# frobelbest/BANet

Measured on AMD Instinct MI355X. Metric: LM iterations/sec (2-frame 640x480 5-level dense BA, 128-coeff depth basis, batch 32), higher is better.
Workload: dtype f32 (SYRK: fp32 operands as bf16x3 / scaled fp16x2 pieces, fp32 accumulate, <= 2e-7 per entry; roofline.syrk_form)

## Files before the change

banet_amd/csrc/gather128s.hip:

```cpp
#include <cstdlib>

#include "quad_common.hpp"
#include "strip_plan.hpp"
static_assert(banet::kStripSegW == banet::kStripW && banet::kStripSegH == banet::kStripH && banet::kStripMinW == banet::kWinTex, "plan.hpp sizes the strip launch by these");

#ifndef BANET_STRIP_OPT_DEFAULT
#define BANET_STRIP_OPT_DEFAULT 0
#endif

namespace banet {

constexpr int kC128s = 128;
constexpr int kSBlock = 128;
constexpr int kSWaves = kSBlock / kWave;
constexpr int kWinFloats = kWinRows * kWinTex * 32;
constexpr int kWinPitchF = kWinTex * 32;

__device__ __forceinline__ int write_lane(int v, int l, int old) { return lane_id() == l ? v : old; }

struct StripLaneEnv {
  int modev, ytv, ybv;
  int ctlv, yfv;
  int ringv;
  __device__ __forceinline__ int mode(int r) const { return __builtin_amdgcn_readlane(modev, r); }
  __device__ __forceinline__ int yt(int r) const { return __builtin_amdgcn_readlane(ytv, r); }
  __device__ __forceinline__ int yb(int r) const { return __builtin_amdgcn_readlane(ybv, r); }
  __device__ __forceinline__ void set_step(int r, int ctl, int yfirst) {
    ctlv = write_lane(ctl, r, ctlv);
    yfv = write_lane(yfirst, r, yfv);
  }
  __device__ __forceinline__ int ring_get(int i) const { return __builtin_amdgcn_readlane(ringv, i); }
  __device__ __forceinline__ void ring_set(int i, int v) { ringv = write_lane(v, i, ringv); }
};

#ifndef BANET_STRIP_NT
#define BANET_STRIP_NT 0
#endif
#if BANET_STRIP_NT >= 2
#define BANET_WIN_NT_ " nt"
#else
#define BANET_WIN_NT_ ""
#endif
__device__ __forceinline__ void glds16(const float* gbase, unsigned voff_bytes, unsigned lds_dst) {
  unsigned keep;
  asm volatile("s_mov_b32 %0, m0\n\ts_mov_b32 m0, %3\n\ts_nop 0\n\tglobal_load_lds_dwordx4 %1, %2" BANET_WIN_NT_ "\n\ts_mov_b32 m0, %0"
               : "=&s"(keep)
               : "v"(voff_bytes), "s"(gbase), "s"(lds_dst)
               : "memory");
}
__device__ __forceinline__ void glds_row(const float* gbase, unsigned v0, unsigned v1, unsigned v2, unsigned lds_dst,
                                         unsigned long long mask3) {
  unsigned keep;
  unsigned long long keepx;
  asm volatile(
      "s_mov_b32 %0, m0\n\ts_mov_b32 m0, %6\n\ts_nop 0\n\t"
      "global_load_lds_dwordx4 %2, %5" BANET_WIN_NT_ "\n\t"
      "global_load_lds_dwordx4 %3, %5 offset:1024" BANET_WIN_NT_ "\n\t"
      "s_mov_b64 %1, exec\n\ts_mov_b64 exec, %7\n\t"
      "global_load_lds_dwordx4 %4, %5 offset:2048" BANET_WIN_NT_ "\n\t"
      "s_mov_b64 exec, %1\n\ts_mov_b32 m0, %0"
      : "=&s"(keep), "=&s"(keepx)
      : "v"(v0), "v"(v1), "v"(v2), "s"(gbase), "s"(lds_dst), "s"(mask3)
      : "memory");
}
template <int N>
__device__ __forceinline__ void wait_vm() {
  asm volatile("s_waitcnt vmcnt(%0)" ::"n"(N) : "memory");
}
__device__ __forceinline__ void wait_vmcnt(int n) {
  if (n >= 8) {
    if (n >= 12) {
      if (n >= 14) wait_vm<14>();
      else wait_vm<12>();
    } else {
      if (n >= 10) wait_vm<10>();
      else wait_vm<8>();
    }
  } else {
    if (n >= 4) {
      if (n >= 6) wait_vm<6>();
      else wait_vm<4>();
    } else {
      if (n >= 2) wait_vm<2>();
      else wait_vm<0>();
    }
  }
}
static_assert(kMaxWait == 15, "wait_vmcnt implements counts up to 15");

constexpr int kStripVgprs = 224;
#if BANET_STRIP_NT >= 1
#define BANET_SRC_NT_ " nt"
#else
#define BANET_SRC_NT_ ""
#endif
#define BANET_SRC_ISSUE_(A0, A1, A2, A3, voff, rs, soff)                                                            \
  asm volatile("buffer_load_dwordx4 v[" #A0 ":" #A3 "], %0, %1, %2 offen" BANET_SRC_NT_ ::"v"(voff), "s"(rs), "s"(soff) \
               : "memory", "v" #A0, "v" #A1, "v" #A2, "v" #A3)
#define BANET_SRC_READ_(A0, A1, A2, A3, d)                                                                          \
  asm volatile("v_mov_b32 %0, v" #A0 "\n\tv_mov_b32 %1, v" #A1 "\n\tv_mov_b32 %2, v" #A2 "\n\tv_mov_b32 %3, v" #A3 \
               : "=v"(d.x), "=v"(d.y), "=v"(d.z), "=v"(d.w))
template <int SLOT, int T>
__device__ __forceinline__ void src_issue(unsigned voff, __amdgpu_buffer_rsrc_t rs, unsigned soff) {
  if constexpr (SLOT == 0 && T == 0) BANET_SRC_ISSUE_(224, 225, 226, 227, voff, rs, soff);
  if constexpr (SLOT == 0 && T == 1) BANET_SRC_ISSUE_(228, 229, 230, 231, voff, rs, soff);
  if constexpr (SLOT == 1 && T == 0) BANET_SRC_ISSUE_(232, 233, 234, 235, voff, rs, soff);
  if constexpr (SLOT == 1 && T == 1) BANET_SRC_ISSUE_(236, 237, 238, 239, voff, rs, soff);
  if constexpr (SLOT == 2 && T == 0) BANET_SRC_ISSUE_(240, 241, 242, 243, voff, rs, soff);
  if constexpr (SLOT == 2 && T == 1) BANET_SRC_ISSUE_(244, 245, 246, 247, voff, rs, soff);
  if constexpr (SLOT == 3 && T == 0) BANET_SRC_ISSUE_(248, 249, 250, 251, voff, rs, soff);
  if constexpr (SLOT == 3 && T == 1) BANET_SRC_ISSUE_(252, 253, 254, 255, voff, rs, soff);
}
template <int SLOT, int T>
__device__ __forceinline__ float4 src_read() {
  float4 d;
  if constexpr (SLOT == 0 && T == 0) BANET_SRC_READ_(224, 225, 226, 227, d);
  if constexpr (SLOT == 0 && T == 1) BANET_SRC_READ_(228, 229, 230, 231, d);
  if constexpr (SLOT == 1 && T == 0) BANET_SRC_READ_(232, 233, 234, 235, d);
  if constexpr (SLOT == 1 && T == 1) BANET_SRC_READ_(236, 237, 238, 239, d);
  if constexpr (SLOT == 2 && T == 0) BANET_SRC_READ_(240, 241, 242, 243, d);
  if constexpr (SLOT == 2 && T == 1) BANET_SRC_READ_(244, 245, 246, 247, d);
  if constexpr (SLOT == 3 && T == 0) BANET_SRC_READ_(248, 249, 250, 251, d);
  if constexpr (SLOT == 3 && T == 1) BANET_SRC_READ_(252, 253, 254, 255, d);
  return d;
}
template <int V>
struct IC {
  static constexpr int value = V;
};

extern __shared__ __attribute__((aligned(16))) float sDynS[];
constexpr int kSWaveLdsFloats = kWinFloats + kC128s;
inline size_t strip_fp_lds_bytes(int pairs, int nch) { return ((size_t)pairs * kSWaveLdsFloats + (size_t)nch * 64 + 4) * sizeof(float); }

template <int KV4, int NCH, bool FP, int OPT = 0>
__global__ __launch_bounds__(FP ? 512 : kSBlock, 2) __attribute__((amdgpu_num_vgpr(kStripVgprs / 2))) void ba_gather128s_kernel(const GatherArgs a) {
  constexpr bool kPipe = (OPT & 1) != 0, kM0Row = (OPT & 2) != 0;
  constexpr int SEGH = 4 * NCH;
  constexpr int NH = (NCH + 3) / 4;
  constexpr int CPG = NCH < 4 ? NCH : 4;
  __shared__ __attribute__((aligned(16))) float sWinS[FP ? 1 : kSWaves][FP ? 4 : kWinFloats];
  __shared__ __attribute__((aligned(16))) float sScrS[FP ? 1 : kSWaves][FP ? 4 : kC128s];
  const banet_level_t& lv = a.lv;
  const int b = blockIdx.y;
  if (a.active != nullptr && a.active[(size_t)b * a.active_stride] == 0) return;
  const int lane = threadIdx.x & 63;
  const int w = wave_id();
  [[maybe_unused]] const int nw = FP ? a.pairs : kSWaves;
  float* const sWinW = FP ? sDynS + (size_t)w * kSWaveLdsFloats : &sWinS[FP ? 0 : w][0];
  float* const sScrW = FP ? sWinW + kWinFloats : &sScrS[FP ? 0 : w][0];
  [[maybe_unused]] float* const sDep = sDynS + (size_t)nw * kSWaveLdsFloats;
  [[maybe_unused]] int* const sItem = reinterpret_cast<int*>(sDep + NCH * 64);
  const int N = lv.N, K = lv.K, H = lv.H, W = lv.W;
  constexpr int C = kC128s;
  const float* __restrict__ src_b = lv.src + (size_t)b * N * C;
  const float* __restrict__ dep_b = lv.depth + (size_t)b * N;
  const float* __restrict__ bas_b = KV4 ? lv.basis + (size_t)b * N * K : nullptr;
  const int nitems = a.tiles, segs_y = a.tiles_y;
  const int pc = lane >> 2, oc = lane & 3, hA = (lane >> 3) & 1;
  const int jA = 4 * hA + oc, jB = 4 * (1 - hA) + oc;
  const int half = lane >> 5, li = lane & 31;
  const unsigned win_base = (unsigned)(uintptr_t)(__attribute__((address_space(3))) float*)sWinW;
  const unsigned dma_off = (unsigned)((lane >> 3) * 512 + (lane & 7) * 16);
  const unsigned srcA_off = (unsigned)(pc * 512 + jA * 16), srcB_off = (unsigned)(pc * 512 + jB * 16);
  StripRowStat* sStat = reinterpret_cast<StripRowStat*>(sScrW);

  float wreg[KV4 ? KV4 : 1][4];
  if constexpr (KV4 > 0) {
#pragma unroll
    for (int kc = 0; kc < KV4; ++kc)
#pragma unroll
      for (int e = 0; e < 4; ++e) {
        const int k = kc * 128 + li * 4 + e;
        wreg[kc][e] = (k < K) ? a.Wc[(size_t)b * K + k] : 0.f;
      }
  }
  [[maybe_unused]] const auto rs_src = __builtin_amdgcn_make_buffer_rsrc(const_cast<float*>(src_b), 0, N * C * 4, 0x00020000);

  int* __restrict__ queue = a.queue + blockIdx.y * 8;
  auto pop_raw = [&]() {
    int v = 0;
    if (lane == 0) v = atomicAdd(&queue[0], 1);
    return v;
  };
  int raw_next = (!FP || w == 0) ? pop_raw() : 0;

  for (int it = 0;; ++it) {
    int wi;
#if defined(BANET_TIMING) && BANET_TIMING == 3
    BANET_TICK(tb0);
#endif
    if constexpr (FP) {
      if (w == 0 && lane == 0) sItem[it & 1] = raw_next;
      __syncthreads();
      wi = rfl(sItem[it & 1]);
    } else {
      wi = rfl(raw_next);
    }
    if (wi >= nitems) return;
    if (!FP || w == 0) raw_next = pop_raw();
    const int sx = wi / segs_y, sy = wi - sx * segs_y;
    const int px = sx * kStripW + pc;
    const int py0 = sy * SEGH + oc;

    BANET_TICK(ts0);
#ifdef BANET_TIMING
    float ts_wait = 0.f;
    [[maybe_unused]] float ts_issue = 0.f, ts_ldsA = 0.f, ts_mathA = 0.f, ts_ldsB = 0.f, ts_mathB = 0.f, ts_bar = 0.f;
#if BANET_TIMING == 3
    ts_bar = (float)(ts0 - tb0);
#endif
#endif
    fvec4 Dv[NH];
    if constexpr (KV4 > 0) {
      constexpr int RB = FP ? (KV4 == 2 ? 4 : 8) : (KV4 == 1 ? 16 : 8), NB = 32 / RB;
      f32x4 bv[2][RB][KV4];
      auto issue_batch = [&](auto bufc, int c, int hb) __attribute__((always_inline)) {
        constexpr int BUF = decltype(bufc)::value;
#pragma unroll
        for (int i = 0; i < RB; ++i) {
          const int ld = half * 32 + brev5s(RB * hb + i);
          const int jx = sx * kStripW + (ld >> 2), jy = sy * SEGH + 4 * c + (ld & 3);
          const bool vj = (jx < W) && (jy < H);
#if defined(BANET_ABLATE_STRIP) && BANET_ABLATE_STRIP >= 2
          const float* row = bas_b + (size_t)(vj ? (jy & 3) * W + (jx & 63) : 0) * K;
#else
          const float* row = bas_b + (size_t)(vj ? jy * W + jx : 0) * K;
#endif
#pragma unroll
          for (int kc = 0; kc < KV4; ++kc) {
            const int k = kc * 128 + li * 4;
            bv[BUF][i][kc] = __builtin_nontemporal_load(reinterpret_cast<const f32x4*>(row + (k < K ? k : 0)));
          }
        }
      };
      auto reduce_batch = [&](auto bufc, float (&pend)[6], int hb) __attribute__((always_inline)) {
        constexpr int BUF = decltype(bufc)::value;
#pragma unroll
        for (int i = 0; i < RB; ++i) {
          float acc = 0.f;
#pragma unroll
          for (int kc = 0; kc < KV4; ++kc)
#pragma unroll
            for (int e = 0; e < 4; ++e) acc = fmaf(bv[BUF][i][kc][e], wreg[kc][e], acc);
          carry_push_s<5, 16>(pend, acc, RB * hb + i);
        }
      };
      if constexpr (FP) {
        if (w < NCH) issue_batch(IC<0>{}, w, 0);
#pragma unroll 1
        for (int c = w; c < NCH; c += nw) {
          const int py = py0 + 4 * c;
          const bool valid = (px < W) && (py < H);
          float D = valid ? dep_b[py * W + px] : 0.f;
          float pend[6];
#pragma unroll
          for (int hb = 0; hb < NB; ++hb) {
            __builtin_amdgcn_sched_barrier(0);
            if (hb + 1 < NB) {
              if ((hb & 1) == 0) issue_batch(IC<1>{}, c, hb + 1);
              else issue_batch(IC<0>{}, c, hb + 1);
            } else if (c + nw < NCH) {
              issue_batch(IC<0>{}, c + nw, 0);
            }
            __builtin_amdgcn_sched_barrier(0);
            if ((hb & 1) == 0) reduce_batch(IC<0>{}, pend, hb);
            else reduce_batch(IC<1>{}, pend, hb);
          }
          sDep[c * 64 + lane] = D + pend[5];
        }
#if defined(BANET_TIMING) && BANET_TIMING == 3
        BANET_TICK(tb2);
#endif
        __syncthreads();
#if defined(BANET_TIMING) && BANET_TIMING == 3
        BANET_TICK(tb3);
        ts_bar += (float)(tb3 - tb2);
#endif
#pragma unroll
        for (int hh = 0; hh < NH; ++hh)
#pragma unroll
          for (int c4 = 0; c4 < CPG; ++c4) Dv[hh][c4] = sDep[(4 * hh + c4) * 64 + lane];
      } else {
      issue_batch(IC<0>{}, 0, 0);
#pragma unroll
      for (int hh = 0; hh < NH; ++hh)
#pragma unroll 1
      for (int c4 = 0; c4 < CPG; ++c4) {
        const int c = 4 * hh + c4;
        const int py = py0 + 4 * c;
        const bool valid = (px < W) && (py < H);
        float D = valid ? dep_b[py * W + px] : 0.f;
        float pend[6];
#pragma unroll
        for (int hb = 0; hb < NB; ++hb) {
          __builtin_amdgcn_sched_barrier(0);
          if (hb + 1 < NB) {
            if ((hb & 1) == 0) issue_batch(IC<1>{}, c, hb + 1);
            else issue_batch(IC<0>{}, c, hb + 1);
          } else if (c < NCH - 1) {
            issue_batch(IC<0>{}, c + 1, 0);
          }
          __builtin_amdgcn_sched_barrier(0);
          if ((hb & 1) == 0) reduce_batch(IC<0>{}, pend, hb);
          else reduce_batch(IC<1>{}, pend, hb);
        }
        D += pend[5];
        Dv[hh][c4] = D;
      }
      }
    } else {
#pragma unroll
      for (int hh = 0; hh < NH; ++hh)
#pragma unroll 1
      for (int c4 = 0; c4 < CPG; ++c4) {
        const int c = 4 * hh + c4;
        const int py = py0 + 4 * c;
        const bool valid = (px < W) && (py < H);
        Dv[hh][c4] = valid ? dep_b[py * W + px] : 0.f;
      }
    }

    BANET_TICK(ts1);
#pragma unroll 1
    for (int pr = FP ? w : 0; pr < (FP ? w + 1 : a.pairs); ++pr) {
      const int vb = b * a.pairs + pr;
      const float* __restrict__ tgt_b = lv.tgt + (size_t)vb * H * W * C;
      float* __restrict__ rec_b = KV4 ? a.rec + (size_t)vb * N * 8 : nullptr;
      float* __restrict__ part = a.partials + ((size_t)vb * nitems + wi) * (kGHdr + C);
      const float* Rm = a.R + vb * 9;
      const float* Tv = a.T + vb * 3;
      const PoseIntr pq = load_pose_intr(lv, b, Rm, Tv);

      ivec4 P0v[NH];
      fvec4 DXv[NH], DYv[NH];
#pragma unroll
      for (int hh = 0; hh < NH; ++hh)
#pragma unroll 1
      for (int c4 = 0; c4 < CPG; ++c4) {
        const int c = 4 * hh + c4;
        const int py = py0 + 4 * c;
        const bool valid = (px < W) && (py < H);
        SGeo ge;
        strip_geometry(lv, pq, valid, px, py, Dv[hh][c4], ge);
        const bool fast = (ge.flags & kPixFast) != 0;
        const int m7 = fast ? (ge.y0 - 1) % kWinRows : 0;
        P0v[hh][c4] = (fast ? (ge.x0 | (ge.y0 << 12)) : 0) | (m7 << 24) | (fast ? (1 << 27) : 0);
        DXv[hh][c4] = ge.dx;
        DYv[hh][c4] = ge.dy;
        const int big = 0x3fffffff;
        int ymn = fast ? ge.y0 : big, ymx = fast ? ge.y0 : -big, xmn = fast ? ge.x0 : big, xmx = fast ? ge.x0 : -big;
#pragma unroll
        for (int sh = 4; sh < 64; sh <<= 1) {
          ymn = min(ymn, __shfl_xor(ymn, sh, 64));
          ymx = max(ymx, __shfl_xor(ymx, sh, 64));
          xmn = min(xmn, __shfl_xor(xmn, sh, 64));
          xmx = max(xmx, __shfl_xor(xmx, sh, 64));
        }
        if (lane < 4) {
          StripRowStat st;
          st.ymin = ymn;
          st.ymax = ymx;
          st.xmin = xmn;
          st.xmax = xmx;
          sStat[4 * c + lane] = st;
        }
      }
      [[maybe_unused]] unsigned long long mask3 = 0;
      int xl, ncol3, plan_ctl, plan_yf;
      {
        StripRowStat st = sStat[lane & (SEGH - 1)];
        if (lane >= SEGH) st.ymin = 1, st.ymax = 0;
        int xm = st.ymin <= st.ymax ? st.xmin : 0x3fffffff;
#pragma unroll
        for (int sh = 1; sh < 64; sh <<= 1) xm = min(xm, __shfl_xor(xm, sh, 64));
        xl = rfl(strip_window_origin(xm, W));
        StripLaneEnv env;
        env.modev = strip_static_mode(st, xl, W);
        env.ytv = st.ymin - 1;
        env.ybv = st.ymax + 2;
        env.ctlv = env.yfv = env.ringv = 0;
        int ye = env.modev == kStepWindow ? env.ybv : -0x3fffffff;
        int xe = env.modev == kStepWindow ? st.xmax + 2 - xl : 0;
#pragma unroll
        for (int sh = 1; sh < 64; sh <<= 1) {
          ye = max(ye, __shfl_xor(ye, sh, 64));
          xe = max(xe, __shfl_xor(xe, sh, 64));
        }
        ncol3 = 8 * max(rfl(xe) + 1 - 16, 1);
        mask3 = ncol3 >= 64 ? ~0ull : ((1ull << ncol3) - 1ull);
        strip_plan_dynamic(env, SEGH, rfl(ye));
        if (lv.flags & kDevStripDirectRows) {
          if (step_mode(env.ctlv) == kStepWindow) env.ctlv = kStepDirect;
        }
        plan_ctl = env.ctlv;
        plan_yf = env.yfv;
      }

      BANET_TICK(ts2);
      fvec4 Q0[NH], Q1[NH], Q2[NH], Q3[NH], Q4[NH];
#pragma unroll
      for (int hh = 0; hh < NH; ++hh) Q0[hh] = Q1[hh] = Q2[hh] = Q3[hh] = Q4[hh] = 0.f;
      const int rowC = W * C;
#pragma unroll 1
      for (int s = 0; s < 4; ++s) {
        float absA[4] = {0.f, 0.f, 0.f, 0.f}, absB[4] = {0.f, 0.f, 0.f, 0.f};
        const float* tgt_s = tgt_b + 32 * s;
#if defined(BANET_ABLATE_STRIP) && BANET_ABLATE_STRIP >= 2
        auto src_soff = [&](int r) { return (unsigned)(((((sy * SEGH + r) & 3) * W + (sx & 3) * kStripW) * C + 32 * s) * 4); };
#else
        auto src_soff = [&](int r) { return (unsigned)((((sy * SEGH + r) * W + sx * kStripW) * C + 32 * s) * 4); };
#endif
        auto issue_row = [&](int Y, int slot) __attribute__((always_inline)) {
#ifdef BANET_ABLATE_STRIP
          const float* gb = tgt_s + ((size_t)(Y & 3) * W + (xl & 15)) * C;
#else
          const float* gb = tgt_s + ((size_t)Y * W + xl) * C;
#endif
          const unsigned dst = win_base + (unsigned)slot * (unsigned)kWinPitchB;
          if constexpr (kM0Row) {
            glds_row(gb, dma_off, dma_off + 3072u, dma_off + 6144u, dst, mask3);
          } else {
            glds16(gb, dma_off, dst);
            glds16(gb + 8 * C, dma_off, dst + 1024u);
            if (lane < ncol3) glds16(gb + 16 * C, dma_off, dst + 2048u);
          }
        };
        asm volatile("s_waitcnt vmcnt(0) lgkmcnt(0)" ::: "memory");
        {
          const int c0 = __builtin_amdgcn_readlane(plan_ctl, 0), c1 = __builtin_amdgcn_readlane(plan_ctl, 1);
          if (step_src_pre(c0)) {
            src_issue<0, 0>(srcA_off, rs_src, src_soff(0));
            src_issue<0, 1>(srcB_off, rs_src, src_soff(0));
          }
          if (step_src_pre(c1)) {
            src_issue<1, 0>(srcA_off, rs_src, src_soff(1));
            src_issue<1, 1>(srcB_off, rs_src, src_soff(1));
          }
        }
#pragma unroll
        for (int hh = 0; hh < NH; ++hh)
#pragma unroll 1
        for (int c4 = 0; c4 < CPG; ++c4) {
          const int c = 4 * hh + c4;
          const int p0c = P0v[hh][c4];
          const float dxc = DXv[hh][c4], dyc = DYv[hh][c4];
          float qacc[5] = {0.f, 0.f, 0.f, 0.f, 0.f};
          auto do_step = [&](auto kconst) __attribute__((always_inline)) {
            constexpr int k = decltype(kconst)::value;
            const int r = 4 * c + k;
            const int ctl = __builtin_amdgcn_readlane(plan_ctl, r);
            const int mode = step_mode(ctl);
            asm volatile("s_waitcnt lgkmcnt(0)" ::: "memory");
#if defined(BANET_TIMING) && BANET_TIMING >= 4
            BANET_TICK(tq0);
#endif
            if (step_src_next(ctl)) {
              src_issue<(k + 2) & 3, 0>(srcA_off, rs_src, src_soff(r + kSrcAhead));
              src_issue<(k + 2) & 3, 1>(srcB_off, rs_src, src_soff(r + kSrcAhead));
            }
            if (mode == kStepSkip) return;
            const int p0 = quad_bcast<k>(p0c);
            const float dx = quad_bcast<k>(dxc), dy = quad_bcast<k>(dyc);
            const bool fast = (p0 >> 27) & 1;
            const float mk = fast ? 1.f : 0.f;
            const float w00 = mk * ((1.f - dx) * (1.f - dy)), w01 = mk * (dx * (1.f - dy)), w10 = mk * ((1.f - dx) * dy),
                        w11 = mk * (dx * dy);
            float qq[5] = {0.f, 0.f, 0.f, 0.f, 0.f};
            if (mode == kStepWindow) {
              const int y0r = __builtin_amdgcn_readlane(plan_yf, r), nr = step_nrows(ctl);
              int slot = y0r % kWinRows;
              for (int i = 0; i < nr; ++i) {
                issue_row(y0r + i, slot);
                slot = slot + 1 == kWinRows ? 0 : slot + 1;
              }
#if defined(BANET_TIMING) && BANET_TIMING == 1
              BANET_TICK(tw0);
#endif
              wait_vmcnt(step_wait(ctl));
#if defined(BANET_TIMING) && BANET_TIMING == 1
              BANET_TICK(tw1);
              BANET_TACC(ts_wait, tw0, tw1);
#endif
              const float4 fA = src_read<k, 0>(), fB = src_read<k, 1>();
              const int mtop = step_mtop(ctl);
              const int xr = fast ? (p0 & 0xfff) - 1 - xl : 0;
              const int m0 = fast ? (p0 >> 24) & 7 : mtop;
              const int m1i = m0 + 1 >= kWinRows ? m0 + 1 - kWinRows : m0 + 1;
              const int m2i = m1i + 1 >= kWinRows ? m1i + 1 - kWinRows : m1i + 1;
              const int m3i = m2i + 1 >= kWinRows ? m2i + 1 - kWinRows : m2i + 1;
              const float* l = sWinW + xr * 32;
              const float* l0 = l + m0 * kWinPitchF;
              const float* l1 = l + m1i * kWinPitchF;
              const float* l2 = l + m2i * kWinPitchF;
              const float* l3 = l + m3i * kWinPitchF;
#if defined(BANET_TIMING) && BANET_TIMING >= 4
              BANET_TICK(tl0);
              [[maybe_unused]] unsigned long long tlm = tl0;
              ts_issue += (float)(tl0 - tq0);
#endif
              if constexpr (kPipe) {
                float4 tA[12], tB[12];
                auto rd = [&](float4 (&t)[12], int po) __attribute__((always_inline)) {
                  t[0] = *reinterpret_cast<const float4*>(l1 + po), t[1] = *reinterpret_cast<const float4*>(l1 + po + 32);
                  t[2] = *reinterpret_cast<const float4*>(l1 + po + 64), t[3] = *reinterpret_cast<const float4*>(l1 + po + 96);
                  t[4] = *reinterpret_cast<const float4*>(l2 + po), t[5] = *reinterpret_cast<const float4*>(l2 + po + 32);
                  t[6] = *reinterpret_cast<const float4*>(l2 + po + 64), t[7] = *reinterpret_cast<const float4*>(l2 + po + 96);
                  t[8] = *reinterpret_cast<const float4*>(l0 + po + 32), t[9] = *reinterpret_cast<const float4*>(l0 + po + 64);
                  t[10] = *reinterpret_cast<const float4*>(l3 + po + 32), t[11] = *reinterpret_cast<const float4*>(l3 + po + 64);
                };
                rd(tA, 4 * jA);
                rd(tB, 4 * jB);
                __builtin_amdgcn_sched_barrier(0);
                tap_math_s(fA, tA[0], tA[1], tA[2], tA[3], tA[4], tA[5], tA[6], tA[7], tA[8], tA[9], tA[10], tA[11], w00, w01, w10, w11, mk, qq, absA);
                __builtin_amdgcn_sched_barrier(0);
                tap_math_s(fB, tB[0], tB[1], tB[2], tB[3], tB[4], tB[5], tB[6], tB[7], tB[8], tB[9], tB[10], tB[11], w00, w01, w10, w11, mk, qq, absB);
              } else {
#pragma unroll
              for (int hp = 0; hp < 2; ++hp) {
                const int po = 4 * (hp ? jB : jA);
                const float4 f1 = hp ? fB : fA;
                const float4 a0 = *reinterpret_cast<const float4*>(l1 + po), a1 = *reinterpret_cast<const float4*>(l1 + po + 32),
                             a2 = *reinterpret_cast<const float4*>(l1 + po + 64), a3 = *reinterpret_cast<const float4*>(l1 + po + 96);
                const float4 b0 = *reinterpret_cast<const float4*>(l2 + po), b1 = *reinterpret_cast<const float4*>(l2 + po + 32),
                             b2 = *reinterpret_cast<const float4*>(l2 + po + 64), b3 = *reinterpret_cast<const float4*>(l2 + po + 96);
                const float4 m1 = *reinterpret_cast<const float4*>(l0 + po + 32), m2 = *reinterpret_cast<const float4*>(l0 + po + 64);
                const float4 p1 = *reinterpret_cast<const float4*>(l3 + po + 32), p2 = *reinterpret_cast<const float4*>(l3 + po + 64);
#if defined(BANET_TIMING) && BANET_TIMING >= 4
                asm volatile("s_waitcnt lgkmcnt(0)" ::: "memory");
                BANET_TICK(tl1);
                if (hp) ts_ldsB += (float)(tl1 - tlm); else ts_ldsA += (float)(tl1 - tl0);
#endif
                if (hp)
                  tap_math_s(f1, a0, a1, a2, a3, b0, b1, b2, b3, m1, m2, p1, p2, w00, w01, w10, w11, mk, qq, absB);
                else
                  tap_math_s(f1, a0, a1, a2, a3, b0, b1, b2, b3, m1, m2, p1, p2, w00, w01, w10, w11, mk, qq, absA);
#if defined(BANET_TIMING) && BANET_TIMING >= 4
                asm volatile("" ::"v"(qq[0]), "v"(qq[4]) : "memory");
                BANET_TICK(tl2);
                if (hp) ts_mathB += (float)(tl2 - tl1); else ts_mathA += (float)(tl2 - tl1);
                tlm = tl2;
#endif
              }
              }
            } else {
              const int x0 = fast ? (p0 & 0xfff) : 1, y0 = fast ? (p0 >> 12) & 0xfff : 1;
              const int gpx = sx * kStripW + pc, gpy = sy * SEGH + r;
              const bool gv = (gpx < W) && (gpy < H);
#pragma unroll
              for (int hp = 0; hp < 2; ++hp) {
                const int po = 32 * s + 4 * (hp ? jB : jA);
                const unsigned osrc = (unsigned)((gv ? gpy * W + gpx : 0) * C + po);
                const unsigned oa = (unsigned)((y0 * W + x0) * C + po);
                const float* ra = tgt_b + (size_t)oa;
                const float* rb = ra + rowC;
                const float* rm = ra - rowC;
                const float* rp = rb + rowC;
                const f32x4 f1v = __builtin_nontemporal_load(reinterpret_cast<const f32x4*>(src_b + (size_t)osrc));
                const float4 f1 = make_float4(f1v[0], f1v[1], f1v[2], f1v[3]);
                const float4 a0 = *reinterpret_cast<const float4*>(ra - C), a1 = *reinterpret_cast<const float4*>(ra),
                             a2 = *reinterpret_cast<const float4*>(ra + C), a3 = *reinterpret_cast<const float4*>(ra + 2 * C);
                const float4 b0 = *reinterpret_cast<const float4*>(rb - C), b1 = *reinterpret_cast<const float4*>(rb),
                             b2 = *reinterpret_cast<const float4*>(rb + C), b3 = *reinterpret_cast<const float4*>(rb + 2 * C);
                const float4 m1 = *reinterpret_cast<const float4*>(rm), m2 = *reinterpret_cast<const float4*>(rm + C);
                const float4 p1 = *reinterpret_cast<const float4*>(rp), p2 = *reinterpret_cast<const float4*>(rp + C);
                if (hp)
                  tap_math_s(f1, a0, a1, a2, a3, b0, b1, b2, b3, m1, m2, p1, p2, w00, w01, w10, w11, mk, qq, absB);
                else
                  tap_math_s(f1, a0, a1, a2, a3, b0, b1, b2, b3, m1, m2, p1, p2, w00, w01, w10, w11, mk, qq, absA);
              }
            }
#pragma unroll
            for (int i = 0; i < 5; ++i) {
              const float tot = quad_sum(qq[i]);
              qacc[i] += (oc == k) ? tot : 0.f;
            }
          };
          do_step(IC<0>{});
          do_step(IC<1>{});
          do_step(IC<2>{});
          do_step(IC<3>{});
          Q0[hh][c4] += qacc[0];
          Q1[hh][c4] += qacc[1];
          Q2[hh][c4] += qacc[2];
          Q3[hh][c4] += qacc[3];
          Q4[hh][c4] += qacc[4];
        }
        asm volatile("s_waitcnt vmcnt(0)" ::: "memory");
#pragma unroll
        for (int e = 0; e < 4; ++e) {
          float lo = hA ? absB[e] : absA[e], hi = hA ? absA[e] : absB[e];
#pragma unroll
          for (int sh = 4; sh < 64; sh <<= 1) {
            lo += __shfl_xor(lo, sh, 64);
            hi += __shfl_xor(hi, sh, 64);
          }
          if (lane < 4) {
            sScrW[32 * s + 4 * oc + e] = lo;
            sScrW[32 * s + 16 + 4 * oc + e] = hi;
          }
        }
      }

      BANET_TICK(ts3);
      float absd2[1][2] = {{0.f, 0.f}};
      float accp[28];
#pragma unroll
      for (int i = 0; i < 28; ++i) accp[i] = 0.f;
#pragma unroll
      for (int hh = 0; hh < NH; ++hh)
#pragma unroll 1
      for (int c4 = 0; c4 < CPG; ++c4) {
        const int c = 4 * hh + c4;
        const int py = py0 + 4 * c;
        const bool valid = (px < W) && (py < H);
        const int pt = valid ? py * W + px : 0;
        SGeo ge;
        strip_geometry(lv, pq, valid, px, py, Dv[hh][c4], ge);
        Q5 qv;
        qv.m11 = Q0[hh][c4];
        qv.m12 = Q1[hh][c4];
        qv.m22 = Q2[hh][c4];
        qv.g1 = Q3[hh][c4];
        qv.g2 = Q4[hh][c4];
        {
          unsigned long long slow = __ballot((ge.flags & kPixRim) != 0);
          while (slow) {
            const int j = __builtin_ctzll(slow);
            slow &= slow - 1;
            const float jdx = rdl(ge.dx, j), jdy = rdl(ge.dy, j);
            Q5 e = border_pixel_q5<2, 1>(rdl(ge.x0, j), rdl(ge.y0, j), (1.f - jdx) * (1.f - jdy), jdx * (1.f - jdy),
                                         (1.f - jdx) * jdy, jdx * jdy, src_b + (size_t)rdl(pt, j) * C, tgt_b, C, H, W, lane,
                                         absd2);
            e.m11 = wave_sum(e.m11);
            e.m12 = wave_sum(e.m12);
            e.m22 = wave_sum(e.m22);
            e.g1 = wave_sum(e.g1);
            e.g2 = wave_sum(e.g2);
            if (lane == j) {
              qv.m11 += e.m11;
              qv.m12 += e.m12;
              qv.m22 += e.m22;
              qv.g1 += e.g1;
              qv.g2 += e.g2;
            }
          }
        }
        const float* jc = ge.jc;
        float mj[12];
#pragma unroll
        for (int i = 0; i < 6; ++i) {
          mj[i] = qv.m11 * jc[i] + qv.m12 * jc[6 + i];
          mj[6 + i] = qv.m12 * jc[i] + qv.m22 * jc[6 + i];
        }
        {
          int o = 0;
#pragma unroll
          for (int i = 0; i < 6; ++i)
#pragma unroll
            for (int jj = i; jj < 6; ++jj) {
              accp[o] += jc[i] * mj[jj] + jc[6 + i] * mj[6 + jj];
              ++o;
            }
#pragma unroll
          for (int i = 0; i < 6; ++i) accp[21 + i] += jc[i] * qv.g1 + jc[6 + i] * qv.g2;
          accp[27] += (float)(ge.flags & kPixInMask);
          if (a.mask_out != nullptr && valid) a.mask_out[(size_t)vb * N + pt] = (unsigned char)(ge.flags & kPixInMask);
        }

        if constexpr (KV4 > 0) {
          if (valid) {
            const float md0 = qv.m11 * ge.jd0 + qv.m12 * ge.jd1, md1 = qv.m12 * ge.jd0 + qv.m22 * ge.jd1;
            float4 ua, ub;
            ua.x = jc[0] * md0 + jc[6] * md1;
            ua.y = jc[1] * md0 + jc[7] * md1;
            ua.z = jc[2] * md0 + jc[8] * md1;
            ua.w = jc[3] * md0 + jc[9] * md1;
            ub.x = jc[4] * md0 + jc[10] * md1;
            ub.y = jc[5] * md0 + jc[11] * md1;
            ub.z = ge.jd0 * md0 + ge.jd1 * md1;
            ub.w = ge.jd0 * qv.g1 + ge.jd1 * qv.g2;
            float4* rp = reinterpret_cast<float4*>(rec_b + (size_t)pt * 8);
            rp[0] = ua;
            rp[1] = ub;
          }
        }
      }
      {
        float pend[6];
#pragma unroll
        for (int i = 0; i < 28; ++i) carry_push_s<5, 32>(pend, accp[i], i);
#pragma unroll
        for (int i = 28; i < 32; ++i) carry_push_s<5, 32>(pend, 0.f, i);
        float tot = pend[5];
        tot += dpp_mov<kDppXor1>(tot);
        const int leaf = brev5s(lane >> 1);
        if ((lane & 1) == 0 && leaf < 28) part[leaf] = tot;
      }
      sScrW[2 * lane] += absd2[0][0];
      sScrW[2 * lane + 1] += absd2[0][1];
      part[kGHdr + lane] = sScrW[lane];
      part[kGHdr + 64 + lane] = sScrW[64 + lane];
#ifdef BANET_TIMING
      {
        BANET_TICK(ts9);
        if (lane == 0) {
#if BANET_TIMING == 1
          part[28] = ts_wait;
          part[29] = (float)(ts3 - ts2);
#elif BANET_TIMING == 3
          part[28] = ts_bar;
          part[29] = (float)(ts2 - ts0) - (ts_bar - (float)(ts0 - tb0));
#elif BANET_TIMING == 4
          part[28] = ts_issue;
          part[29] = ts_ldsA + ts_ldsB;
#elif BANET_TIMING == 5
          part[28] = ts_mathA + ts_mathB;
          part[29] = (float)(ts3 - ts2) - (ts_issue + ts_ldsA + ts_ldsB + ts_mathA + ts_mathB);
#else
          part[28] = (float)(ts1 - ts0);
          part[29] = (float)(ts2 - ts1);
#endif
#if BANET_TIMING >= 4
          part[30] = (float)(ts3 - ts2);
#else
          part[30] = (float)(ts9 - ts3);
#endif
#if BANET_TIMING == 3
          part[31] = (float)(ts9 - tb0);
#else
          part[31] = (float)(ts9 - ts0);
#endif
        }
      }
#endif
    }
  }
}

static int strip_opt() {
  static const int v = [] {
    const char* e = std::getenv("BANET_STRIP_OPT");
    const int x = e ? std::atoi(e) : BANET_STRIP_OPT_DEFAULT;
    return x >= 0 && x <= 3 ? x : 0;
  }();
  return v;
}

int launch_gather128s(const GatherArgs& a, int K, hipStream_t s) {
  dim3 grid(a.G, a.lv.B), block(kSBlock);
  const bool tall = a.seg_h == 32, low = a.seg_h == 8;
  if (a.seg_h != 32 && a.seg_h != 16 && a.seg_h != 8) return BANET_ERR_INVALID_ARG;
  if (a.strip_fp) {
    if (tall || low || a.pairs < 2 || a.pairs > 7) return BANET_ERR_INVALID_ARG;
    const size_t shm = strip_fp_lds_bytes(a.pairs, 4);
    block = dim3(64 * a.pairs);
#define BANET_LAUNCH_FP(KV4)                                                                                              \
  do {                                                                                                                    \
    if (shm > 64 * 1024)                                                                                                  \
      (void)hipFuncSetAttribute(reinterpret_cast<const void*>(&ba_gather128s_kernel<KV4, 4, true>),                       \
                                hipFuncAttributeMaxDynamicSharedMemorySize, (int)shm);                                    \
    hipLaunchKernelGGL((ba_gather128s_kernel<KV4, 4, true>), grid, block, shm, s, a);                                     \
  } while (0)
#define BANET_LAUNCH_FPO(OPT)                                                                                             \
  do {                                                                                                                    \
    if (shm > 64 * 1024)                                                                                                  \
      (void)hipFuncSetAttribute(reinterpret_cast<const void*>(&ba_gather128s_kernel<1, 4, true, OPT>),                    \
                                hipFuncAttributeMaxDynamicSharedMemorySize, (int)shm);                                    \
    hipLaunchKernelGGL((ba_gather128s_kernel<1, 4, true, OPT>), grid, block, shm, s, a);                                  \
  } while (0)
    [[maybe_unused]] const int opt = strip_opt();
    if (K == 0) BANET_LAUNCH_FP(0);
#ifdef BANET_STRIP_OPT_VARIANTS
    else if ((K & 3) == 0 && K <= 128 && opt == 1) BANET_LAUNCH_FPO(1);
    else if ((K & 3) == 0 && K <= 128 && opt == 2) BANET_LAUNCH_FPO(2);
    else if ((K & 3) == 0 && K <= 128 && opt == 3) BANET_LAUNCH_FPO(3);
#endif
    else if ((K & 3) == 0 && K <= 128) BANET_LAUNCH_FP(1);
    else if ((K & 3) == 0 && K <= 256) BANET_LAUNCH_FP(2);
    else return BANET_ERR_UNSUPPORTED;
#undef BANET_LAUNCH_FP
#undef BANET_LAUNCH_FPO
    return BANET_OK;
  }
#define BANET_LAUNCH_S(KV4)                                                                     \
  do {                                                                                          \
    if (tall) hipLaunchKernelGGL((ba_gather128s_kernel<KV4, 8, false>), grid, block, 0, s, a);  \
    else if (low) hipLaunchKernelGGL((ba_gather128s_kernel<KV4, 2, false>), grid, block, 0, s, a); \
    else hipLaunchKernelGGL((ba_gather128s_kernel<KV4, 4, false>), grid, block, 0, s, a);       \
  } while (0)
  [[maybe_unused]] const int opt = strip_opt();
  if (K == 0) BANET_LAUNCH_S(0);
#ifdef BANET_STRIP_OPT_VARIANTS
  else if ((K & 3) == 0 && K <= 128 && !tall && !low && opt == 1) hipLaunchKernelGGL((ba_gather128s_kernel<1, 4, false, 1>), grid, block, 0, s, a);
  else if ((K & 3) == 0 && K <= 128 && !tall && !low && opt == 2) hipLaunchKernelGGL((ba_gather128s_kernel<1, 4, false, 2>), grid, block, 0, s, a);
  else if ((K & 3) == 0 && K <= 128 && !tall && !low && opt == 3) hipLaunchKernelGGL((ba_gather128s_kernel<1, 4, false, 3>), grid, block, 0, s, a);
#endif
  else if ((K & 3) == 0 && K <= 128) BANET_LAUNCH_S(1);
  else if ((K & 3) == 0 && K <= 256) BANET_LAUNCH_S(2);
  else return BANET_ERR_UNSUPPORTED;
#undef BANET_LAUNCH_S
  return BANET_OK;
}

}
```

banet_amd/csrc/quad_common.hpp:

```cpp
#pragma once
#include "gather_common.hpp"

namespace banet {

typedef float fvec4 __attribute__((ext_vector_type(4)));
typedef int ivec4 __attribute__((ext_vector_type(4)));
typedef float v2fs __attribute__((ext_vector_type(2)));

__device__ __forceinline__ int brev5s(int t) { return (int)(__brev((unsigned)t) >> 27); }

template <int NL, int S0>
__device__ __forceinline__ void carry_push_s(float (&pend)[NL + 1], float v, int t) {
  bool done = false;
#pragma unroll
  for (int L = 0; L < NL; ++L) {
    if (!done) {
      if (((t >> L) & 1) == 0) {
        pend[L] = v;
        done = true;
      } else {
        v = bfly_merge(pend[L], v, S0 >> L);
      }
    }
  }
  if (!done) pend[NL] = v;
}

__device__ __forceinline__ void tap_math_s(const float4& f1, const float4& a0, const float4& a1, const float4& a2,
                                           const float4& a3, const float4& b0, const float4& b1, const float4& b2,
                                           const float4& b3, const float4& m1, const float4& m2, const float4& p1,
                                           const float4& p2, float w00, float w01, float w10, float w11, float mk,
                                           float (&q)[5], float (&absd)[4]) {
  const float h00 = 0.5f * w00, h01 = 0.5f * w01, h10 = 0.5f * w10, h11 = 0.5f * w11;
#ifdef BANET_TAP_SCALAR
  {
    const float F1[4] = {f1.x, f1.y, f1.z, f1.w}, A0[4] = {a0.x, a0.y, a0.z, a0.w}, A1[4] = {a1.x, a1.y, a1.z, a1.w},
                A2[4] = {a2.x, a2.y, a2.z, a2.w}, A3[4] = {a3.x, a3.y, a3.z, a3.w}, B0[4] = {b0.x, b0.y, b0.z, b0.w},
                B1[4] = {b1.x, b1.y, b1.z, b1.w}, B2[4] = {b2.x, b2.y, b2.z, b2.w}, B3[4] = {b3.x, b3.y, b3.z, b3.w},
                M1[4] = {m1.x, m1.y, m1.z, m1.w}, M2[4] = {m2.x, m2.y, m2.z, m2.w}, P1[4] = {p1.x, p1.y, p1.z, p1.w},
                P2[4] = {p2.x, p2.y, p2.z, p2.w};
    float s11[4], s12[4], s22[4], sg1[4], sg2[4];
#pragma unroll
    for (int c = 0; c < 4; ++c) {
      const float f = ((A1[c] * w00 + A2[c] * w01) + B1[c] * w10) + B2[c] * w11;
      const float gx = (((A2[c] - A0[c]) * h00 + (A3[c] - A1[c]) * h01) + (B2[c] - B0[c]) * h10) + (B3[c] - B1[c]) * h11;
      const float gy = (((B1[c] - M1[c]) * h00 + (B2[c] - M2[c]) * h01) + (P1[c] - A1[c]) * h10) + (P2[c] - A2[c]) * h11;
      const float d = f - F1[c] * mk;
      s11[c] = gx * gx, s12[c] = gx * gy, s22[c] = gy * gy, sg1[c] = gx * d, sg2[c] = gy * d;
      absd[c] += fabsf(d);
    }
    q[0] += (s11[0] + s11[2]) + (s11[1] + s11[3]);
    q[1] += (s12[0] + s12[2]) + (s12[1] + s12[3]);
    q[2] += (s22[0] + s22[2]) + (s22[1] + s22[3]);
    q[3] += (sg1[0] + sg1[2]) + (sg1[1] + sg1[3]);
    q[4] += (sg2[0] + sg2[2]) + (sg2[1] + sg2[3]);
    return;
  }
#endif
  v2fs qm11 = {0.f, 0.f}, qm12 = {0.f, 0.f}, qm22 = {0.f, 0.f}, qg1 = {0.f, 0.f}, qg2 = {0.f, 0.f};
#define BANET_V2S(v, k) (v2fs){(k) ? (v).z : (v).x, (k) ? (v).w : (v).y}
#pragma unroll
  for (int k = 0; k < 2; ++k) {
    const v2fs F1 = BANET_V2S(f1, k);
    const v2fs A0 = BANET_V2S(a0, k), A1 = BANET_V2S(a1, k), A2 = BANET_V2S(a2, k), A3 = BANET_V2S(a3, k);
    const v2fs B0 = BANET_V2S(b0, k), B1 = BANET_V2S(b1, k), B2 = BANET_V2S(b2, k), B3 = BANET_V2S(b3, k);
    const v2fs M1 = BANET_V2S(m1, k), M2 = BANET_V2S(m2, k), P1 = BANET_V2S(p1, k), P2 = BANET_V2S(p2, k);
    const v2fs f = ((A1 * w00 + A2 * w01) + B1 * w10) + B2 * w11;
    const v2fs gx = (((A2 - A0) * h00 + (A3 - A1) * h01) + (B2 - B0) * h10) + (B3 - B1) * h11;
    const v2fs gy = (((B1 - M1) * h00 + (B2 - M2) * h01) + (P1 - A1) * h10) + (P2 - A2) * h11;
    const v2fs d = f - F1 * mk;
    qm11 += gx * gx;
    qm12 += gx * gy;
    qm22 += gy * gy;
    qg1 += gx * d;
    qg2 += gy * d;
    absd[2 * k] += fabsf(d.x);
    absd[2 * k + 1] += fabsf(d.y);
  }
#undef BANET_V2S
  q[0] += qm11.x + qm11.y;
  q[1] += qm12.x + qm12.y;
  q[2] += qm22.x + qm22.y;
  q[3] += qg1.x + qg1.y;
  q[4] += qg2.x + qg2.y;
}

__device__ __forceinline__ float quad_sum(float v) {
  v += dpp_mov<kDppXor1>(v);
  v += dpp_mov<kDppXor2>(v);
  return v;
}
template <int K4>
__device__ __forceinline__ int quad_bcast(int v) {
  return __builtin_amdgcn_update_dpp(0, v, K4 * 0x55, 0xF, 0xF, true);
}
template <int K4>
__device__ __forceinline__ float quad_bcast(float v) {
  return __builtin_bit_cast(float, quad_bcast<K4>(__builtin_bit_cast(int, v)));
}

struct SGeo {
  float dx, dy, jd0, jd1;
  float jc[12];
  int x0, y0, flags;
};

struct PoseIntr {
  float R[9], T[3], fx0, fy0, ox0, oy0;
};
__device__ __forceinline__ PoseIntr load_pose_intr(const banet_level_t& lv, int b, const float* __restrict__ Rm, const float* __restrict__ Tv) {
  auto u = [](float v) { return __builtin_bit_cast(float, __builtin_amdgcn_readfirstlane(__builtin_bit_cast(int, v))); };
  PoseIntr q;
#pragma unroll
  for (int i = 0; i < 9; ++i) q.R[i] = u(Rm[i]);
#pragma unroll
  for (int i = 0; i < 3; ++i) q.T[i] = u(Tv[i]);
  q.fx0 = u(lv.intr[b * 4 + 0]);
  q.fy0 = u(lv.intr[b * 4 + 1]);
  q.ox0 = u(lv.intr[b * 4 + 2]);
  q.oy0 = u(lv.intr[b * 4 + 3]);
  return q;
}
__device__ __forceinline__ void strip_geometry(const banet_level_t& lv, const PoseIntr& pq, bool valid, int px, int py, float D, SGeo& o) {
  const int W = lv.W, H = lv.H;
  const float* Rm = pq.R;
  const float* Tv = pq.T;
  o.dx = o.dy = o.jd0 = o.jd1 = 0.f;
  float p0 = 0.f, p1 = 0.f, p2 = 1.f, fx = 1.f, fy = 1.f, ox = 0.f, oy = 0.f;
  if (valid) {
    const float fx0 = pq.fx0, fy0 = pq.fy0, ox0 = pq.ox0, oy0 = pq.oy0;
    p0 = ((float)px * lv.scale - ox0) / fx0;
    p1 = ((float)py * lv.scale - oy0) / fy0;
    p2 = 1.f;
    if (lv.normalize_rays) {
      const float ss = p0 * p0 + p1 * p1 + p2 * p2;
      const float inv = 1.f / sqrtf(fmaxf(ss, 1e-12f));
      p0 *= inv;
      p1 *= inv;
      p2 *= inv;
    }
    fx = fx0 / lv.scale;
    fy = fy0 / lv.scale;
    ox = ox0 / lv.scale;
    oy = oy0 / lv.scale;
  }
  const float rx = Rm[0] * p0 + Rm[1] * p1 + Rm[2] * p2;
  const float ry = Rm[3] * p0 + Rm[4] * p1 + Rm[5] * p2;
  const float rz = Rm[6] * p0 + Rm[7] * p1 + Rm[8] * p2;
  const float X = rx * D + Tv[0], Y = ry * D + Tv[1], Z = rz * D + Tv[2];
  const float x = X / Z, y = Y / Z;
  const float pxl = fx * x + ox, pyl = fy * y + oy;
  const bool m = valid && (pxl >= 0.f) && (pxl <= (float)(W - 1)) && (pyl >= 0.f) && (pyl <= (float)(H - 1));
#pragma unroll
  for (int i = 0; i < 12; ++i) o.jc[i] = 0.f;
  int x0 = 0, y0 = 0;
  if (m) {
    const float xf = floorf(pxl), yf = floorf(pyl);
    o.dx = pxl - xf;
    o.dy = pyl - yf;
    x0 = (int)xf;
    y0 = (int)yf;
    const float iz = 1.f / Z;
    o.jc[0] = fx * (x * y);
    o.jc[1] = fx * (-1.f - x * x);
    o.jc[2] = fx * y;
    o.jc[3] = fx * (-iz);
    o.jc[4] = 0.f;
    o.jc[5] = fx * (x / Z);
    o.jc[6] = fy * (1.f + y * y);
    o.jc[7] = fy * (-(x * y));
    o.jc[8] = fy * (-x);
    o.jc[9] = 0.f;
    o.jc[10] = fy * (-iz);
    o.jc[11] = fy * (y / Z);
    o.jd0 = fx * ((rx - rz * x) / Z);
    o.jd1 = fy * ((ry - rz * y) / Z);
  }
  const bool interior = (x0 >= 1) && (x0 + 2 <= W - 1) && (y0 >= 1) && (y0 + 2 <= H - 1);
  const bool fast = m && interior;
  o.flags = (m ? kPixInMask : 0) | (fast ? kPixFast : 0) | ((m && !fast) ? kPixRim : 0);
  o.x0 = x0;
  o.y0 = y0;
}

}
```

Baseline: 26310.

## Fold quad reductions across steps and precompute window tap offsets

Each step of the strip gather used to run a full quad_sum butterfly on its five accumulators and then mask the result to the owning lane. The new default path keeps separate accumulators for step pairs and merges them with transpose-style fold1/fold2 DPP operations, so four steps take fewer shuffles and selects. It also rewrites P0 once per strip with pre-subtracted column offsets (or mtop for slow pixels) and computes LDS row addresses with a wraparound trick based on unsigned min, and it forces the pair horizontal sum to be a single add. The old behaviour stays available through a BANET_STRIP_LEGACY_STEP environment variable, at the cost of doubling template instantiations and adding more live registers for the paired accumulators.

```diff
diff --git a/banet_amd/csrc/gather128s.hip b/banet_amd/csrc/gather128s.hip
--- a/banet_amd/csrc/gather128s.hip
+++ b/banet_amd/csrc/gather128s.hip
@@ -135,7 +135,7 @@
 
 template <int KV4, int NCH, bool FP, int OPT = 0>
 __global__ __launch_bounds__(FP ? 512 : kSBlock, 2) __attribute__((amdgpu_num_vgpr(kStripVgprs / 2))) void ba_gather128s_kernel(const GatherArgs a) {
-  constexpr bool kPipe = (OPT & 1) != 0, kM0Row = (OPT & 2) != 0;
+  constexpr bool kPipe = (OPT & 1) != 0, kM0Row = (OPT & 2) != 0, kLegacy = (OPT & 4) != 0;
   constexpr int SEGH = 4 * NCH;
   constexpr int NH = (NCH + 3) / 4;
   constexpr int CPG = NCH < 4 ? NCH : 4;
@@ -396,6 +396,16 @@
         plan_ctl = env.ctlv;
         plan_yf = env.yfv;
       }
+      if constexpr (!kLegacy) {
+#pragma unroll
+        for (int hh = 0; hh < NH; ++hh)
+#pragma unroll
+          for (int c4 = 0; c4 < CPG; ++c4) {
+            const int ctl_r = __shfl(plan_ctl, 4 * (4 * hh + c4) + oc, 64);
+            const int p = P0v[hh][c4];
+            P0v[hh][c4] = ((p >> 27) & 1) ? ((p & ~0xfff) | ((p - 1 - xl) & 0xfff)) : (step_mtop(ctl_r) << 24);
+          }
+      }
 
       BANET_TICK(ts2);
       fvec4 Q0[NH], Q1[NH], Q2[NH], Q3[NH], Q4[NH];
@@ -445,8 +455,8 @@
           const int c = 4 * hh + c4;
           const int p0c = P0v[hh][c4];
           const float dxc = DXv[hh][c4], dyc = DYv[hh][c4];
-          float qacc[5] = {0.f, 0.f, 0.f, 0.f, 0.f};
-          auto do_step = [&](auto kconst) __attribute__((always_inline)) {
+          [[maybe_unused]] float qacc[5] = {0.f, 0.f, 0.f, 0.f, 0.f};
+          auto do_step = [&](auto kconst, float (&qq)[5]) __attribute__((always_inline)) {
             constexpr int k = decltype(kconst)::value;
             const int r = 4 * c + k;
             const int ctl = __builtin_amdgcn_readlane(plan_ctl, r);
@@ -466,7 +476,6 @@
             const float mk = fast ? 1.f : 0.f;
             const float w00 = mk * ((1.f - dx) * (1.f - dy)), w01 = mk * (dx * (1.f - dy)), w10 = mk * ((1.f - dx) * dy),
                         w11 = mk * (dx * dy);
-            float qq[5] = {0.f, 0.f, 0.f, 0.f, 0.f};
             if (mode == kStepWindow) {
               const int y0r = __builtin_amdgcn_readlane(plan_yf, r), nr = step_nrows(ctl);
               int slot = y0r % kWinRows;
@@ -483,17 +492,30 @@
               BANET_TACC(ts_wait, tw0, tw1);
 #endif
               const float4 fA = src_read<k, 0>(), fB = src_read<k, 1>();
-              const int mtop = step_mtop(ctl);
-              const int xr = fast ? (p0 & 0xfff) - 1 - xl : 0;
-              const int m0 = fast ? (p0 >> 24) & 7 : mtop;
-              const int m1i = m0 + 1 >= kWinRows ? m0 + 1 - kWinRows : m0 + 1;
-              const int m2i = m1i + 1 >= kWinRows ? m1i + 1 - kWinRows : m1i + 1;
-              const int m3i = m2i + 1 >= kWinRows ? m2i + 1 - kWinRows : m2i + 1;
-              const float* l = sWinW + xr * 32;
-              const float* l0 = l + m0 * kWinPitchF;
-              const float* l1 = l + m1i * kWinPitchF;
-              const float* l2 = l + m2i * kWinPitchF;
-              const float* l3 = l + m3i * kWinPitchF;
+              [[maybe_unused]] const int mtop = step_mtop(ctl);
+              const float *l0, *l1, *l2, *l3;
+              if constexpr (kLegacy) {
+                const int xr = fast ? (p0 & 0xfff) - 1 - xl : 0;
+                const int m0 = fast ? (p0 >> 24) & 7 : mtop;
+                const int m1i = m0 + 1 >= kWinRows ? m0 + 1 - kWinRows : m0 + 1;
+                const int m2i = m1i + 1 >= kWinRows ? m1i + 1 - kWinRows : m1i + 1;
+                const int m3i = m2i + 1 >= kWinRows ? m2i + 1 - kWinRows : m2i + 1;
+                const float* l = sWinW + xr * 32;
+                l0 = l + m0 * kWinPitchF;
+                l1 = l + m1i * kWinPitchF;
+                l2 = l + m2i * kWinPitchF;
+                l3 = l + m3i * kWinPitchF;
+              } else {
+                constexpr unsigned kP = (unsigned)kWinPitchB;
+                static_assert((kWinTex - 1) * 128 < kWinPitchB, "the wrap needs column offsets below the pitch");
+                const unsigned t0 = (unsigned)((p0 >> 24) & 7) * kP + ((unsigned)(p0 & 0xfff) << 7);
+                const unsigned t1 = min(t0 + kP, t0 - 6u * kP), t2 = min(t1 + kP, t1 - 6u * kP), t3 = min(t2 + kP, t2 - 6u * kP);
+                const char* lw = reinterpret_cast<const char*>(sWinW);
+                l0 = reinterpret_cast<const float*>(lw + t0);
+                l1 = reinterpret_cast<const float*>(lw + t1);
+                l2 = reinterpret_cast<const float*>(lw + t2);
+                l3 = reinterpret_cast<const float*>(lw + t3);
+              }
 #if defined(BANET_TIMING) && BANET_TIMING >= 4
               BANET_TICK(tl0);
               [[maybe_unused]] unsigned long long tlm = tl0;
@@ -512,9 +534,9 @@
                 rd(tA, 4 * jA);
                 rd(tB, 4 * jB);
                 __builtin_amdgcn_sched_barrier(0);
-                tap_math_s(fA, tA[0], tA[1], tA[2], tA[3], tA[4], tA[5], tA[6], tA[7], tA[8], tA[9], tA[10], tA[11], w00, w01, w10, w11, mk, qq, absA);
+                tap_math_s<!kLegacy>(fA, tA[0], tA[1], tA[2], tA[3], tA[4], tA[5], tA[6], tA[7], tA[8], tA[9], tA[10], tA[11], w00, w01, w10, w11, mk, qq, absA);
                 __builtin_amdgcn_sched_barrier(0);
-                tap_math_s(fB, tB[0], tB[1], tB[2], tB[3], tB[4], tB[5], tB[6], tB[7], tB[8], tB[9], tB[10], tB[11], w00, w01, w10, w11, mk, qq, absB);
+                tap_math_s<!kLegacy>(fB, tB[0], tB[1], tB[2], tB[3], tB[4], tB[5], tB[6], tB[7], tB[8], tB[9], tB[10], tB[11], w00, w01, w10, w11, mk, qq, absB);
               } else {
 #pragma unroll
               for (int hp = 0; hp < 2; ++hp) {
@@ -532,9 +554,9 @@
                 if (hp) ts_ldsB += (float)(tl1 - tlm); else ts_ldsA += (float)(tl1 - tl0);
 #endif
                 if (hp)
-                  tap_math_s(f1, a0, a1, a2, a3, b0, b1, b2, b3, m1, m2, p1, p2, w00, w01, w10, w11, mk, qq, absB);
+                  tap_math_s<!kLegacy>(f1, a0, a1, a2, a3, b0, b1, b2, b3, m1, m2, p1, p2, w00, w01, w10, w11, mk, qq, absB);
                 else
-                  tap_math_s(f1, a0, a1, a2, a3, b0, b1, b2, b3, m1, m2, p1, p2, w00, w01, w10, w11, mk, qq, absA);
+                  tap_math_s<!kLegacy>(f1, a0, a1, a2, a3, b0, b1, b2, b3, m1, m2, p1, p2, w00, w01, w10, w11, mk, qq, absA);
 #if defined(BANET_TIMING) && BANET_TIMING >= 4
                 asm volatile("" ::"v"(qq[0]), "v"(qq[4]) : "memory");
                 BANET_TICK(tl2);
@@ -544,7 +566,7 @@
               }
               }
             } else {
-              const int x0 = fast ? (p0 & 0xfff) : 1, y0 = fast ? (p0 >> 12) & 0xfff : 1;
+              const int x0 = fast ? ((p0 + (kLegacy ? 0 : xl + 1)) & 0xfff) : 1, y0 = fast ? (p0 >> 12) & 0xfff : 1;
               const int gpx = sx * kStripW + pc, gpy = sy * SEGH + r;
               const bool gv = (gpx < W) && (gpy < H);
 #pragma unroll
@@ -565,21 +587,36 @@
                 const float4 m1 = *reinterpret_cast<const float4*>(rm), m2 = *reinterpret_cast<const float4*>(rm + C);
                 const float4 p1 = *reinterpret_cast<const float4*>(rp), p2 = *reinterpret_cast<const float4*>(rp + C);
                 if (hp)
-                  tap_math_s(f1, a0, a1, a2, a3, b0, b1, b2, b3, m1, m2, p1, p2, w00, w01, w10, w11, mk, qq, absB);
+                  tap_math_s<!kLegacy>(f1, a0, a1, a2, a3, b0, b1, b2, b3, m1, m2, p1, p2, w00, w01, w10, w11, mk, qq, absB);
                 else
-                  tap_math_s(f1, a0, a1, a2, a3, b0, b1, b2, b3, m1, m2, p1, p2, w00, w01, w10, w11, mk, qq, absA);
+                  tap_math_s<!kLegacy>(f1, a0, a1, a2, a3, b0, b1, b2, b3, m1, m2, p1, p2, w00, w01, w10, w11, mk, qq, absA);
               }
             }
-#pragma unroll
-            for (int i = 0; i < 5; ++i) {
-              const float tot = quad_sum(qq[i]);
-              qacc[i] += (oc == k) ? tot : 0.f;
+            if constexpr (kLegacy) {
+#pragma unroll
+              for (int i = 0; i < 5; ++i) {
+                const float tot = quad_sum(qq[i]);
+                qacc[i] += (oc == k) ? tot : 0.f;
+              }
             }
           };
-          do_step(IC<0>{});
-          do_step(IC<1>{});
-          do_step(IC<2>{});
-          do_step(IC<3>{});
+          float qa[5] = {0.f, 0.f, 0.f, 0.f, 0.f}, qb[5] = {0.f, 0.f, 0.f, 0.f, 0.f};
+          do_step(IC<0>{}, qa);
+          do_step(IC<1>{}, qb);
+          if constexpr (kLegacy) {
+#pragma unroll
+            for (int i = 0; i < 5; ++i) qa[i] = qb[i] = 0.f;
+            do_step(IC<2>{}, qa);
+            do_step(IC<3>{}, qb);
+          } else {
+            float p01[5];
+#pragma unroll
+            for (int i = 0; i < 5; ++i) p01[i] = quad_fold1(qa[i], qb[i]), qa[i] = qb[i] = 0.f;
+            do_step(IC<2>{}, qa);
+            do_step(IC<3>{}, qb);
+#pragma unroll
+            for (int i = 0; i < 5; ++i) qacc[i] = quad_fold2(p01[i], quad_fold1(qa[i], qb[i]));
+          }
           Q0[hh][c4] += qacc[0];
           Q1[hh][c4] += qacc[1];
           Q2[hh][c4] += qacc[2];
@@ -746,8 +783,13 @@
   }();
   return v;
 }
-
-int launch_gather128s(const GatherArgs& a, int K, hipStream_t s) {
+static bool strip_legacy_step() {
+  const char* e = std::getenv("BANET_STRIP_LEGACY_STEP");
+  return e != nullptr && e[0] == '1';
+}
+
+template <int LG>
+static int launch_gather128s_t(const GatherArgs& a, int K, hipStream_t s) {
   dim3 grid(a.G, a.lv.B), block(kSBlock);
   const bool tall = a.seg_h == 32, low = a.seg_h == 8;
   if (a.seg_h != 32 && a.seg_h != 16 && a.seg_h != 8) return BANET_ERR_INVALID_ARG;
@@ -755,26 +797,20 @@
     if (tall || low || a.pairs < 2 || a.pairs > 7) return BANET_ERR_INVALID_ARG;
     const size_t shm = strip_fp_lds_bytes(a.pairs, 4);
     block = dim3(64 * a.pairs);
-#define BANET_LAUNCH_FP(KV4)                                                                                              \
+#define BANET_LAUNCH_FPO(KV4, OPT)                                                                                        \
   do {                                                                                                                    \
     if (shm > 64 * 1024)                                                                                                  \
-      (void)hipFuncSetAttribute(reinterpret_cast<const void*>(&ba_gather128s_kernel<KV4, 4, true>),                       \
+      (void)hipFuncSetAttribute(reinterpret_cast<const void*>(&ba_gather128s_kernel<KV4, 4, true, OPT>),                  \
                                 hipFuncAttributeMaxDynamicSharedMemorySize, (int)shm);                                    \
-    hipLaunchKernelGGL((ba_gather128s_kernel<KV4, 4, true>), grid, block, shm, s, a);                                     \
+    hipLaunchKernelGGL((ba_gather128s_kernel<KV4, 4, true, OPT>), grid, block, shm, s, a);                                \
   } while (0)
-#define BANET_LAUNCH_FPO(OPT)                                                                                             \
-  do {                                                                                                                    \
-    if (shm > 64 * 1024)                                                                                                  \
-      (void)hipFuncSetAttribute(reinterpret_cast<const void*>(&ba_gather128s_kernel<1, 4, true, OPT>),                    \
-                                hipFuncAttributeMaxDynamicSharedMemorySize, (int)shm);                                    \
-    hipLaunchKernelGGL((ba_gather128s_kernel<1, 4, true, OPT>), grid, block, shm, s, a);                                  \
-  } while (0)
+#define BANET_LAUNCH_FP(KV4) BANET_LAUNCH_FPO(KV4, LG)
     [[maybe_unused]] const int opt = strip_opt();
     if (K == 0) BANET_LAUNCH_FP(0);
 #ifdef BANET_STRIP_OPT_VARIANTS
-    else if ((K & 3) == 0 && K <= 128 && opt == 1) BANET_LAUNCH_FPO(1);
-    else if ((K & 3) == 0 && K <= 128 && opt == 2) BANET_LAUNCH_FPO(2);
-    else if ((K & 3) == 0 && K <= 128 && opt == 3) BANET_LAUNCH_FPO(3);
+    else if ((K & 3) == 0 && K <= 128 && opt == 1) BANET_LAUNCH_FPO(1, LG | 1);
+    else if ((K & 3) == 0 && K <= 128 && opt == 2) BANET_LAUNCH_FPO(1, LG | 2);
+    else if ((K & 3) == 0 && K <= 128 && opt == 3) BANET_LAUNCH_FPO(1, LG | 3);
 #endif
     else if ((K & 3) == 0 && K <= 128) BANET_LAUNCH_FP(1);
     else if ((K & 3) == 0 && K <= 256) BANET_LAUNCH_FP(2);
@@ -783,18 +819,18 @@
 #undef BANET_LAUNCH_FPO
     return BANET_OK;
   }
-#define BANET_LAUNCH_S(KV4)                                                                     \
-  do {                                                                                          \
-    if (tall) hipLaunchKernelGGL((ba_gather128s_kernel<KV4, 8, false>), grid, block, 0, s, a);  \
-    else if (low) hipLaunchKernelGGL((ba_gather128s_kernel<KV4, 2, false>), grid, block, 0, s, a); \
-    else hipLaunchKernelGGL((ba_gather128s_kernel<KV4, 4, false>), grid, block, 0, s, a);       \
+#define BANET_LAUNCH_S(KV4)                                                                          \
+  do {                                                                                               \
+    if (tall) hipLaunchKernelGGL((ba_gather128s_kernel<KV4, 8, false, LG>), grid, block, 0, s, a);   \
+    else if (low) hipLaunchKernelGGL((ba_gather128s_kernel<KV4, 2, false, LG>), grid, block, 0, s, a); \
+    else hipLaunchKernelGGL((ba_gather128s_kernel<KV4, 4, false, LG>), grid, block, 0, s, a);        \
   } while (0)
   [[maybe_unused]] const int opt = strip_opt();
   if (K == 0) BANET_LAUNCH_S(0);
 #ifdef BANET_STRIP_OPT_VARIANTS
-  else if ((K & 3) == 0 && K <= 128 && !tall && !low && opt == 1) hipLaunchKernelGGL((ba_gather128s_kernel<1, 4, false, 1>), grid, block, 0, s, a);
-  else if ((K & 3) == 0 && K <= 128 && !tall && !low && opt == 2) hipLaunchKernelGGL((ba_gather128s_kernel<1, 4, false, 2>), grid, block, 0, s, a);
-  else if ((K & 3) == 0 && K <= 128 && !tall && !low && opt == 3) hipLaunchKernelGGL((ba_gather128s_kernel<1, 4, false, 3>), grid, block, 0, s, a);
+  else if ((K & 3) == 0 && K <= 128 && !tall && !low && opt == 1) hipLaunchKernelGGL((ba_gather128s_kernel<1, 4, false, LG | 1>), grid, block, 0, s, a);
+  else if ((K & 3) == 0 && K <= 128 && !tall && !low && opt == 2) hipLaunchKernelGGL((ba_gather128s_kernel<1, 4, false, LG | 2>), grid, block, 0, s, a);
+  else if ((K & 3) == 0 && K <= 128 && !tall && !low && opt == 3) hipLaunchKernelGGL((ba_gather128s_kernel<1, 4, false, LG | 3>), grid, block, 0, s, a);
 #endif
   else if ((K & 3) == 0 && K <= 128) BANET_LAUNCH_S(1);
   else if ((K & 3) == 0 && K <= 256) BANET_LAUNCH_S(2);
@@ -803,4 +839,8 @@
   return BANET_OK;
 }
 
-}
+int launch_gather128s(const GatherArgs& a, int K, hipStream_t s) {
+  return strip_legacy_step() ? launch_gather128s_t<4>(a, K, s) : launch_gather128s_t<0>(a, K, s);
+}
+
+}
diff --git a/banet_amd/csrc/quad_common.hpp b/banet_amd/csrc/quad_common.hpp
--- a/banet_amd/csrc/quad_common.hpp
+++ b/banet_amd/csrc/quad_common.hpp
@@ -26,6 +26,13 @@
   if (!done) pend[NL] = v;
 }
 
+__device__ __forceinline__ float hsum2(v2fs v) {
+  float r;
+  asm("v_add_f32 %0, %1, %2" : "=v"(r) : "v"(v.x), "v"(v.y));
+  return r;
+}
+
+template <bool HS = false>
 __device__ __forceinline__ void tap_math_s(const float4& f1, const float4& a0, const float4& a1, const float4& a2,
                                            const float4& a3, const float4& b0, const float4& b1, const float4& b2,
                                            const float4& b3, const float4& m1, const float4& m2, const float4& p1,
@@ -78,6 +85,14 @@
     absd[2 * k + 1] += fabsf(d.y);
   }
 #undef BANET_V2S
+  if constexpr (HS) {
+    q[0] += hsum2(qm11);
+    q[1] += hsum2(qm12);
+    q[2] += hsum2(qm22);
+    q[3] += hsum2(qg1);
+    q[4] += hsum2(qg2);
+    return;
+  }
   q[0] += qm11.x + qm11.y;
   q[1] += qm12.x + qm12.y;
   q[2] += qm22.x + qm22.y;
@@ -89,6 +104,14 @@
   v += dpp_mov<kDppXor1>(v);
   v += dpp_mov<kDppXor2>(v);
   return v;
+}
+__device__ __forceinline__ float quad_fold1(float a, float b) {
+  const bool odd = (lane_id() & 1) != 0;
+  return (odd ? b : a) + dpp_mov<kDppXor1>(odd ? a : b);
+}
+__device__ __forceinline__ float quad_fold2(float p, float q) {
+  const bool hi = (lane_id() & 2) != 0;
+  return (hi ? q : p) + dpp_mov<kDppXor2>(hi ? p : q);
 }
 template <int K4>
 __device__ __forceinline__ int quad_bcast(int v) {
```

After: 26160. No clear change (-0.6%).
